# deep-art-project/Music

Hardware: AMD Instinct MI355X
Metric: audio samples/sec trained (whole node), 30-layer WaveNet @16kHz (higher is better)
Workload: dtype f32 (forward + recompute: f16 2-term split operands, 2^-22 per element; backward products: bf16 2-term split, 2^-17 per element, f32 range; 3 MFMA per product, f32 accumulate)

## Files before the change

### include/wavenet_hip.h

```cpp
#ifndef WAVENET_HIP_H
#define WAVENET_HIP_H
#include <stdint.h>
#ifdef __cplusplus
extern "C" {
#endif

typedef void* wn_stream_t;
enum { WN_F16X3 = 0, WN_F16X1 = 1, WN_BF16X3 = 2, WN_BF16X1 = 3 };
#define WN_ABI_VERSION 9
#define WN_CE_NUM_PARTIALS 1024
#define WN_GUARD_NUM_PARTIALS 256
#define WN_GUARD_PARTIALS_BYTES (WN_GUARD_NUM_PARTIALS * 12)
#define WN_GUARD_STATE_BYTES 48

int wn_version(void);
const char* wn_last_error(void);

int wn_pack_weights(const float* flat, const int32_t* idx, uint16_t* out, int n, int mode,
                    wn_stream_t stream);

int wn_chan_gemm(const float* in0, const float* in1, int64_t in_bstride, int in_pitch, int in_lo, int in_hi,
                 int shift0, int shift1, int ks0, int ks1, const uint16_t* wpack, int mt, int m_valid,
                 float* out, int64_t out_bstride, int out_pitch, int out_shift, const float* bias,
                 const float* resid, int64_t resid_bstride, int resid_pitch, int resid_lo,
// ... 27 lines not shown

int wn_enc_resblock_fwd(const float* x_in, float* x_out, float* h_out, int64_t x_bstride, int64_t h_bstride, int pitch,
                        const uint16_t* wdil, const uint16_t* wd, const float* bias_dil, const float* bias_d, int n_h,
                        int n_d, int ch, int d, int t_lo, int t_hi, int batch, int mode, wn_stream_t stream);

int wn_enc_resblock_bwd(const float* x_in, const float* dy, const float* h, float* dh, int64_t x_bstride,
                        int64_t h_bstride, int64_t dh_bstride, int pitch, const uint16_t* wdT, int ch, int d, int t_lo,
                        int t_hi, int y_lo, float* slab_dil, float* slab_d, int batch, int mode_bwd, wn_stream_t stream);
int wn_enc_resblock_bwd_slabs(int t_lo, int t_hi, int batch);
int wn_enc_resblock_bwd_pq(const float* x_in, const float* p_in, const float* q_in, int dn, int p_lo, const float* h,
                           float* p_out, float* q_out, int64_t x_bstride, int64_t h_bstride, int pitch, const uint16_t* wdT,
                           const uint16_t* wpq, int ch, int d, int t_lo, int t_hi, float* slab_dil, float* slab_d, int chain,
                           int batch, int mode_bwd, wn_stream_t stream);

int wn_resblock_bwd_ms(const float* x_in, const float* dy, const float* dz, float* dfg, int64_t x_bstride,
                       int64_t dz_bstride, int64_t dfg_bstride, int pitch, const uint16_t* wfg, const uint16_t* wdT,
                       const float* bias_f, const float* bias_g, int n_f, int ch, int d, int t_lo, int t_hi, int z_lo,
                       float* slab_fg, float* slab_d, const float* cond, int64_t cond_bstride, int cond_pitch,
                       int cond_mode, int cond_le, int cond_q, int batch, int mode_fwd, int mode_bwd,
                       wn_stream_t stream);
int wn_resblock_bwd_ms_slabs(int t_lo, int t_hi, int batch);

#define WN_COND_IDX_PAD 64
int wn_resblock_bwd_pq(const float* x_in, const float* p_in, const float* q_in, int dn, int p_lo, const float* dz,
                       float* p_out, float* q_out, int64_t x_bstride, int64_t dz_bstride, int pitch, const uint16_t* wfg,
                       const uint16_t* wdT, const uint16_t* wpq, int ch, int d, int t_lo, int t_hi, int z_lo,
                       float* slab_fg, float* slab_d, const float* cond, int64_t cond_bstride, int cond_pitch, int cond_le,
                       const uint8_t* cond_idx, float* cslab, int64_t dz_half_stride, int chain, int batch, int mode_fwd,
                       int mode_bwd, wn_stream_t stream);
int wn_resblock_bwd_pq_chain_ok(int t_lo, int t_hi, int batch, int d);
int wn_resblock_bwd_pq_slabs(int t_lo, int t_hi, int batch, int d, int chain);
int wn_resblock_bwd_pq_chain_items(int t_lo, int t_hi, int batch, int d, int wg, int* out, int cap);
int wn_resblock_bwd_pq_cond_floats(int t_lo, int t_hi, int batch);
int wn_resblock_bwd_pq_cond_reduce(const float* cslab, const int64_t* slab_off, const int* t_lo, int n_launches, int t_hi, int batch,
                                   int cond_le, float* out, int64_t out_lstride, int64_t out_bstride, int out_pitch,
                                   wn_stream_t stream);
int wn_gate_fwd(const float* fg, int64_t fg_bstride, int dp, int rows, float* z, int64_t z_bstride, int pitch, int t_lo, int t_hi,
                int batch, wn_stream_t stream);
int wn_gate_bwd(const float* fg, int64_t fg_bstride, int dp, int rows, const float* dz, int64_t dz_bstride, float* dfg,
                int64_t dfg_bstride, int pitch, int t_lo, int t_hi, int batch, wn_stream_t stream);
int wn_chunk_softmax_fwd(const float* x, float* y, int64_t nrows, int q, wn_stream_t stream);
int wn_chunk_softmax_bwd(const float* y, const float* dy, float* dx, int64_t nrows, int q, wn_stream_t stream);
int wn_chunk_softmax_ce(const float* x, const int64_t* target, float* probs, float* dx, float* loss_part, int64_t nrows, int q,
                        float inv_n, wn_stream_t stream);
int wn_split16(const float* x, uint16_t* hi, uint16_t* lo, int64_t n, int is_bf16, wn_stream_t stream);
int wn_shift_add(const float* p, const float* q, float* out, int64_t bstride, int pitch, int rows, int dn, int p_lo,
                 int t_lo, int t_hi, int batch, wn_stream_t stream);

int wn_wgrad(const float* a, int64_t a_bstride, int a_pitch, int a_shift, int a_cols,
             const float* b0, const float* b1, int64_t b_bstride, int b_pitch, int b_shift0,
             int b_shift1, int b_cols, int nt_per_tap, int mt, int relu_b, float* c, int ldc,
             int64_t c_slab_stride, int t_lo, int t_hi, int chunk, int batch, int mode, wn_stream_t stream);
int wn_wgrad_slabs(int t_lo, int t_hi, int chunk, int batch);
int wn_causal_wgrad_codes(const int32_t* codes, int scrambled, const float* dx, const float* dx_q, int dn, int p_lo,
                          int64_t dx_bstride, int pitch, int ch, int q, int t, int batch, float* slab, wn_stream_t stream);
int wn_causal_wgrad_codes_slabs(int t, int batch);
int wn_causal_fwd_codes(const int32_t* codes, int scrambled, const float* wt, const float* bias, int n_rows, float* x0,
                        int64_t x_bstride, int pitch, int ch, int q, int t, int batch, wn_stream_t stream);
int wn_reduce_slabs(const int64_t* desc, int n_ops, int64_t total_vec, const float* slab, float* out,
                    wn_stream_t stream);

int wn_bias_grad(const float* a, int64_t a_bstride, int a_pitch, int a_shift, int rows, int t_lo,
                 int t_hi, int batch, float* out, wn_stream_t stream);

int wn_chunk_softmax256_fwd(const float* x, float* y, int64_t nrows, wn_stream_t stream);
int wn_chunk_softmax256_bwd(const float* y, const float* dy, float* dx, int64_t nrows, wn_stream_t stream);
int wn_chunk_softmax256_ce(const float* x, const int64_t* target, float* probs, float* dx,
                           float* loss_part, int64_t nrows, float inv_n, wn_stream_t stream);

int wn_adam_flat(float* p, const float* g, float* m, float* v, int64_t n, float lr, float beta1,
                 float beta2, float eps, float bias_corr1, float bias_corr2, float gscale,
                 wn_stream_t stream);
int wn_sgd_flat(float* p, const float* g, float* momentum_buf, int64_t n, float lr, float momentum, float gscale,
                int first_step, wn_stream_t stream);
int wn_rmsprop_flat(float* p, const float* g, float* square_avg, float* momentum_buf, int64_t n, float lr, float alpha,
                    float eps, float momentum, float gscale, wn_stream_t stream);
typedef struct wn_guard_state {
    float norm;
    float coef;
    uint32_t nonfinite;
    uint32_t skip;
    uint64_t n_taken;
    uint64_t n_clipped;
    uint64_t n_skipped;
    float bc1;
    float bc2;
} wn_guard_state;
int wn_grad_guard(const float* g, int64_t n, float gscale, float max_norm, int skip_nonfinite, float beta1, float beta2,
                  void* partials, wn_guard_state* state, wn_stream_t stream);
int wn_adam_flat_guarded(float* p, const float* g, float* m, float* v, int64_t n, float lr, float beta1, float beta2, float eps,
                         float gscale, const wn_guard_state* state, wn_stream_t stream);
int wn_sgd_flat_guarded(float* p, const float* g, float* momentum_buf, int64_t n, float lr, float momentum, float gscale,
                        const wn_guard_state* state, wn_stream_t stream);
int wn_rmsprop_flat_guarded(float* p, const float* g, float* square_avg, float* momentum_buf, int64_t n, float lr, float alpha,
                            float eps, float momentum, float gscale, const wn_guard_state* state, wn_stream_t stream);
int wn_ema_flat(float* ema, const float* p, int64_t n, float decay, int warmup, int64_t t, const wn_guard_state* state,
                wn_stream_t stream);
int wn_step_softmax(const float* x, int64_t x_bstride, int x_pitch, float* probs, int w, int q, int batch, wn_stream_t stream);
int wn_step_nll(const float* x, int64_t x_bstride, int x_pitch, const int64_t* target, float* dx, int64_t dx_bstride, int dx_pitch,
                float* probs, float* row_nll, int32_t* row_hit, float* loss_part, int w, int q, int batch, float inv_n,
                wn_stream_t stream);
int wn_win_step_softmax(const float* x, int64_t x_bstride, int x_pitch, float* probs, int w, int q, int batch, const int32_t* win_host,
                        int win_period, const int64_t* win_pos, int64_t win_pos0, wn_stream_t stream);
int wn_win_step_nll(const float* x, int64_t x_bstride, int x_pitch, const int64_t* target, float* dx, int64_t dx_bstride, int dx_pitch,
                    float* probs, float* row_nll, int32_t* row_hit, float* loss_part, int w, int q, int batch, float inv_n,
                    const int32_t* win_host, int win_period, const int64_t* win_pos, int64_t win_pos0, wn_stream_t stream);
// ... 155 lines not shown
```

### music_amd/_lib.py

```python
import ctypes
import os

_HERE = os.path.dirname(os.path.abspath(__file__))
LIB_PATH = os.environ.get("WAVENET_HIP_LIB") or os.path.join(_HERE, "libwavenet_hip.so")

F16X3, F16X1, BF16X3, BF16X1 = 0, 1, 2, 3
MODE_NAMES = {"f16x3": F16X3, "f16x1": F16X1, "bf16x3": BF16X3, "bf16x1": BF16X1}
CE_NUM_PARTIALS = 1024
ABI_VERSION = 9
GUARD_NUM_PARTIALS = 256
GUARD_PARTIALS_BYTES = GUARD_NUM_PARTIALS * 12
VQ_NUM_PARTIALS = 256
VQ_MAX_CODES, VQ_MAX_WIDTH = 1024, 512
VQ_EMA_WORK_BYTES = 16 + 4 * VQ_MAX_CODES
RVQ_MAX_STAGES = 8
GCOND_MAX_CHANNELS = 512

_p = ctypes.c_void_p
_i = ctypes.c_int
_l = ctypes.c_int64
_f = ctypes.c_float
_DEC_HEAD = [_i] * 5 + [_p] * 6 + [_l] + [_p] * 12 + [_l, _i, _i, _p]
_DEC_BATCH = [_i, _l, _f, _l]
_DEC_PK = [_p] + [_l] * 6
_DEC_COND = [_p, _l, _p, _l, _p, _p, _i, _l]
_DEC_SAMP = [_p, _i, _f]
_DEC_WIN = [_p, _i, _l]
_SAMPLE_LOGITS = [_p, _l, _i, _l, _p, _f, _l, _i, _f, _l, _p, _p, _p]

SIGNATURES = {
    "wn_version": [],
    "wn_pack_weights": [_p, _p, _p, _i, _i, _p],
    "wn_chan_gemm": [_p, _p, _l, _i, _i, _i, _i, _i, _i, _i, _p, _i, _i,
                     _p, _l, _i, _i, _p,
                     _p, _l, _i, _i,
                     _p, _l, _i,
                     _i, _i, _i, _i, _i, _p],
    "wn_skip_epilogue_fwd": [_p, _l, _i, _i, _p, _p, _p, _p, _l, _p, _p, _p, _p, _p, _l, _i, _i, _i, _i, _i, _i, _i, _p],
    "wn_skip_epilogue_bwd": [_p, _l, _i, _p, _p, _l, _i, _p, _p, _p, _l, _p, _p, _p, _i, _i, _i, _i, _i, _i, _i, _p],
    "wn_resblock_fwd": [_p, _p, _p, _l, _l, _i, _p, _p, _p, _p, _p, _i, _i, _i, _i,
                        _i, _i, _i, _i, _p, _l, _i, _i, _i, _i, _p, _l, _p, _l, _i, _i, _p],
    "wn_enc_resblock_fwd": [_p, _p, _p, _l, _l, _i, _p, _p, _p, _p, _i, _i, _i, _i, _i, _i, _i, _i, _p],
    "wn_enc_resblock_bwd": [_p, _p, _p, _p, _l, _l, _l, _i, _p, _i, _i, _i, _i, _i, _p, _p, _i, _i, _p],
    "wn_enc_resblock_bwd_slabs": [_i, _i, _i],
    "wn_enc_resblock_bwd_pq": [_p, _p, _p, _i, _i, _p, _p, _p, _l, _l, _i, _p, _p, _i, _i, _i, _i, _p, _p, _i, _i, _i, _p],
    "wn_avgpool": [_p, _l, _i, _i, _i, _i, _i, _p, _l, _i, _i, _p],
    "wn_resblock_bwd": [_p, _p, _p, _p, _p, _l, _l, _l, _l, _i, _p, _p, _p, _p, _i, _i, _i, _i, _i, _i,
                        _p, _l, _i, _i, _i, _i, _i, _i, _i, _p],
    "wn_cond_expand": [_p, _l, _i, _i, _i, _i, _i, _i, _i, _p, _l, _i, _i, _p],
    "wn_cond_grad": [_p, _l, _i, _i, _i, _i, _i, _i, _i, _p, _l, _i, _i, _p],
    "wn_avgpool_bwd": [_p, _l, _i, _i, _i, _i, _i, _p, _l, _i, _i, _i, _p],
    "wn_wgrad": [_p, _l, _i, _i, _i, _p, _p, _l, _i, _i, _i, _i, _i, _i, _i, _p, _i,
                 _l, _i, _i, _i, _i, _i, _p],
    "wn_wgrad_slabs": [_i, _i, _i, _i],
    "wn_resblock_bwd_ms": [_p, _p, _p, _p, _l, _l, _l, _i, _p, _p, _p, _p, _i, _i, _i, _i, _i, _i, _p, _p,
                           _p, _l, _i, _i, _i, _i, _i, _i, _i, _p],
    "wn_resblock_bwd_ms_slabs": [_i, _i, _i],
    "wn_resblock_bwd_pq": [_p, _p, _p, _i, _i, _p, _p, _p, _l, _l, _i, _p, _p, _p, _i, _i, _i, _i, _i, _p, _p,
                           _p, _l, _i, _i, _p, _p, _l, _i, _i, _i, _i, _p],
    "wn_resblock_bwd_pq_chain_ok": [_i, _i, _i, _i],
    "wn_resblock_bwd_pq_slabs": [_i, _i, _i, _i, _i],
    "wn_resblock_bwd_pq_chain_items": [_i, _i, _i, _i, _i, _p, _i],
    "wn_resblock_bwd_pq_cond_floats": [_i, _i, _i],
    "wn_resblock_bwd_pq_cond_reduce": [_p, _p, _p, _i, _i, _i, _i, _p, _l, _l, _i, _p],
    "wn_split16": [_p, _p, _p, _l, _i, _p],
    "wn_shift_add": [_p, _p, _p, _l, _i, _i, _i, _i, _i, _i, _i, _p],
    "wn_causal_wgrad_codes": [_p, _i, _p, _p, _i, _i, _l, _i, _i, _i, _i, _i, _p, _p],
    "wn_causal_wgrad_codes_slabs": [_i, _i],
    "wn_causal_fwd_codes": [_p, _i, _p, _p, _i, _p, _l, _i, _i, _i, _i, _i, _p],
    "wn_reduce_slabs": [_p, _i, _l, _p, _p, _p],
    "wn_bias_grad": [_p, _l, _i, _i, _i, _i, _i, _i, _p, _p],
    "wn_chunk_softmax256_fwd": [_p, _p, _l, _p],
    "wn_chunk_softmax256_bwd": [_p, _p, _p, _l, _p],
    "wn_chunk_softmax256_ce": [_p, _p, _p, _p, _p, _l, _f, _p],
    "wn_gate_fwd": [_p, _l, _i, _i, _p, _l, _i, _i, _i, _i, _p],
    "wn_gate_bwd": [_p, _l, _i, _i, _p, _l, _p, _l, _i, _i, _i, _i, _p],
    "wn_chunk_softmax_fwd": [_p, _p, _l, _i, _p],
    "wn_chunk_softmax_bwd": [_p, _p, _p, _l, _i, _p],
    "wn_chunk_softmax_ce": [_p, _p, _p, _p, _p, _l, _i, _f, _p],
    "wn_adam_flat": [_p, _p, _p, _p, _l, _f, _f, _f, _f, _f, _f, _f, _p],
    "wn_sgd_flat": [_p, _p, _p, _l, _f, _f, _f, _i, _p],
    "wn_rmsprop_flat": [_p, _p, _p, _p, _l, _f, _f, _f, _f, _f, _p],
    "wn_grad_guard": [_p, _l, _f, _f, _i, _f, _f, _p, _p, _p],
    "wn_adam_flat_guarded": [_p, _p, _p, _p, _l, _f, _f, _f, _f, _f, _p, _p],
    "wn_sgd_flat_guarded": [_p, _p, _p, _l, _f, _f, _f, _p, _p],
    "wn_rmsprop_flat_guarded": [_p, _p, _p, _p, _l, _f, _f, _f, _f, _f, _p, _p],
    "wn_ema_flat": [_p, _p, _l, _f, _i, _l, _p, _p],
    "wn_step_softmax": [_p, _l, _i, _p, _i, _i, _i, _p],
    "wn_step_nll": [_p, _l, _i, _p, _p, _l, _i, _p, _p, _p, _p, _i, _i, _i, _f, _p],
    "wn_win_step_softmax": [_p, _l, _i, _p, _i, _i, _i, _p, _i, _p, _l, _p],
    "wn_win_step_nll": [_p, _l, _i, _p, _p, _l, _i, _p, _p, _p, _p, _i, _i, _i, _f, _p, _i, _p, _l, _p],
    "wn_cond_proj_fwd": [_p, _p, _l, _l, _l, _l, _l, _p, _p, _p, _i, _i, _i, _i, _i, _i, _i, _p],
    "wn_cond_proj_bwd": [_p, _i, _p, _p, _p, _l, _l, _l, _l, _l, _p, _p, _i, _i, _i, _i, _i, _i, _i, _p],
    "wn_gcond_proj_fwd": [_p, _p, _l, _l, _l, _l, _l, _p, _p, _p, _i, _i, _i, _i, _i, _i, _i, _p, _l, _l, _l, _l, _i, _i, _p],
    "wn_gcond_proj_bwd": [_p, _i, _p, _p, _p, _l, _l, _l, _l, _l, _p, _p, _i, _i, _i, _i, _i, _i, _i, _p, _l, _l, _l, _l, _i, _i, _p],
    "wn_vq_fwd": [_p, _p, _l, _p, _p, _p, _p, _i, _i, _i, _i, _p],
    "wn_vq_bwd": [_p, _p, _p, _p, _l, _f, _f, _p, _p, _i, _i, _i, _i, _p],
    "wn_vq_lookup": [_p, _p, _l, _p, _p, _i, _i, _i, _i, _p],
    "wn_vq_bwd_stats": [_p, _p, _p, _p, _l, _f, _f, _p, _p, _p, _i, _i, _i, _i, _p],
    "wn_vq_ema_update": [_p, _l, _p, _p, _p, _p, _i, _i, _f, _f, _f, _p, _p],
    "wn_rvq_fwd": [_p, _p, _l, _p, _p, _p, _p, _p, _i, _i, _i, _i, _i, _p],
    "wn_rvq_bwd": [_p, _p, _p, _p, _p, _l, _f, _f, _p, _p, _i, _i, _i, _i, _i, _p],
    "wn_rvq_bwd_stats": [_p, _p, _p, _p, _p, _l, _f, _f, _p, _p, _p, _i, _i, _i, _i, _i, _p],
    "wn_rvq_ema_update": [_p, _l, _p, _p, _p, _p, _i, _i, _i, _f, _f, _f, _p, _p],
    "wn_rvq_lookup": [_p, _p, _l, _p, _p, _i, _i, _i, _i, _i, _i, _p],
    "wn_rvq_fwd_n": [_p, _p, _l, _p, _p, _p, _p, _p, _p, _i, _i, _i, _i, _i, _p],
    "wn_rvq_bwd_n": [_p, _p, _p, _p, _p, _p, _l, _f, _f, _p, _p, _i, _i, _i, _i, _i, _p],
# ... 85 lines not shown
def thread_budget(quota, local_world, cpus=None):
    total = quota if quota is not None else (cpus if cpus is not None else (os.cpu_count() or 1))
    return max(1, -(-int(total) // max(1, int(local_world))))


def respect_cpu_quota():
    import sys
    import torch
    if os.environ.get("WN_KEEP_TORCH_THREADS", "0") == "1":
        return
    q, lw = cpu_quota(), local_world_size()
    if q is None and lw == 1:
        return
    n = thread_budget(q, lw)
    if torch.get_num_threads() > n:
        print("music_amd: torch intra-op threads %d -> %d (%s shared by %d rank(s) of this host; WN_KEEP_TORCH_THREADS=1 keeps torch's "
              "own setting)" % (torch.get_num_threads(), n, "the container's CPU quota of %d" % q if q is not None else
                                "%d CPUs" % (os.cpu_count() or 1), lw), file=sys.stderr)
        torch.set_num_threads(n)


def load():
    global _lib
    if _lib is not None:
        return _lib
    if not os.path.exists(LIB_PATH):
        raise WavenetHipError(
            "libwavenet_hip.so not found at %s - build it with `python -c 'import __graft_entry__ as g; "
            "g.build()'` or `make -C music_amd/csrc`; there is no CPU fallback" % LIB_PATH)
    import torch
    lib = ctypes.CDLL(LIB_PATH)
    for name, args in SIGNATURES.items():
        try:
            fn = getattr(lib, name)
        except AttributeError:
            raise WavenetHipError("%s does not export %s: it was built from older sources - rebuild it (`make -C music_amd/csrc`)"
                                  % (LIB_PATH, name)) from None
        fn.argtypes = args
        fn.restype = ctypes.c_int
    lib.wn_decode_sync_granules.restype = ctypes.c_int64
    lib.wn_last_error.argtypes = []
    lib.wn_last_error.restype = ctypes.c_char_p
    if lib.wn_version() != ABI_VERSION:
        raise WavenetHipError("libwavenet_hip.so ABI version %d != expected %d" % (lib.wn_version(), ABI_VERSION))
    _lib = lib
    respect_cpu_quota()
    return lib


def wgrad_slabs(t_lo, t_hi, chunk, batch):
    return load().wn_wgrad_slabs(t_lo, t_hi, chunk, batch)


def causal_codes_slabs(t, batch):
    return load().wn_causal_wgrad_codes_slabs(t, batch)


COND_IDX_PAD = 64


def ms_slabs(t_lo, t_hi, batch):
    return load().wn_resblock_bwd_ms_slabs(t_lo, t_hi, batch)


def pq_chain_ok(t_lo, t_hi, batch, d):
    return bool(load().wn_resblock_bwd_pq_chain_ok(t_lo, t_hi, batch, d))


def pq_slabs(t_lo, t_hi, batch, d, chain):
    return load().wn_resblock_bwd_pq_slabs(t_lo, t_hi, batch, d, 1 if chain else 0)


def enc_slabs(t_lo, t_hi, batch):
    return load().wn_enc_resblock_bwd_slabs(t_lo, t_hi, batch)


def decode_sync_granules(n_layers, D, S):
    return int(load().wn_decode_sync_granules(n_layers, D, S))


def call(name, *args):
    lib = load()
    rc = getattr(lib, name)(*args)
    if rc != 0:
        raise WavenetHipError("%s failed (%d): %s" % (name, rc, lib.wn_last_error().decode()))


def ptr(t, offset=0):
    if t is None:
        return None
    return t.data_ptr() + offset * t.element_size()


def stream():
    import torch
    return torch.cuda.current_stream().cuda_stream


_side_streams = {}


def side_stream(device):
    import os
    import torch
    dev = torch.device(device)
    key = dev.index if dev.index is not None else torch.cuda.current_device()
# ... 5 lines not shown
```

### music_amd/csrc/wn_api.hip

```cpp
#include <stdio.h>
#include <stdlib.h>
#include <string.h>
#include "../../include/wavenet_hip.h"
#include "wn_common.h"
#include "wn_kernels.h"

static_assert(WN_COND_IDX_PAD == WN_PQ_IDX_PAD, "public and kernel-side pad of the bucket bytes differ");
static thread_local char g_err[512] = "";

int wn_set_error(hipError_t e, const char* file, int line) {
    snprintf(g_err, sizeof(g_err), "HIP error %d (%s) at %s:%d", (int)e, hipGetErrorString(e), file, line);
    return -1;
}
int wn_tile_origin(int t_lo) { return t_lo & ~63; }

int wn_num_cus() {
    static std::atomic<int> cus{0};
    int v = cus.load(std::memory_order_relaxed);
    if (v > 0) return v;
    int dev = 0;
    hipDeviceProp_t pr;
    if (hipGetDevice(&dev) != hipSuccess || hipGetDeviceProperties(&pr, dev) != hipSuccess || pr.multiProcessorCount <= 0) return 256;
    cus.store(pr.multiProcessorCount, std::memory_order_relaxed);
    return pr.multiProcessorCount;
// ... 247 lines not shown
        if (write_x) WN_REQUIRE("wn_resblock_fwd", x_out);
    }
    WnResArgs a;
    memset(&a, 0, sizeof(a));
    a.x_in = x_in; a.x_out = x_out; a.z_out = z_out; a.x_bstride = x_bstride; a.z_bstride = z_bstride; a.pitch = pitch;
    a.wfg = wfg; a.wd = wd; a.bias_f = bias_f; a.bias_g = bias_g; a.bias_d = bias_d; a.n_f = n_f; a.n_d = n_d;
    a.d = d; a.t_lo = t_lo; a.t_hi = t_hi; a.z_lo = z_lo; a.write_x = write_x;
    a.cond = cond; a.cond_bstride = cond_bstride; a.cond_pitch = cond_pitch; a.cond_mode = cond_mode;
    a.cond_le = cond_le; a.cond_q = cond_q;
    if (cond && cond_pack && cond_idx) { a.cond_pack = cond_pack; a.cond_pack_bstride = cond_pack_bstride; a.cond_idx = cond_idx; }
    if (z_half_stride && ch != 64) return wn_set_error_msg(-4, "wn_resblock_fwd: z_half_stride is for two 32-channel clips on the 64-channel block");
    a.z_half = z_half_stride;
    return wn_launch_resblock_fwd(a, ch, batch, mode, (hipStream_t)stream);
}

int wn_resblock_bwd(const float* x_in, const float* dy, const float* dz, float* dfg, float* z,
                    int64_t x_bstride, int64_t dz_bstride, int64_t dfg_bstride, int64_t z_bstride,
                    int pitch, const uint16_t* wfg, const uint16_t* wdT, const float* bias_f,
                    const float* bias_g, int n_f, int ch, int d, int t_lo, int t_hi, int z_lo,
                    const float* cond, int64_t cond_bstride, int cond_pitch, int cond_mode, int cond_le, int cond_q,
                    int batch, int mode_fwd, int mode_bwd, wn_stream_t stream) {
    if (pitch % 4 != 0) return wn_set_error_msg(-4, "wn_resblock_bwd: pitch must be a multiple of 4");
    if (batch > 0 && t_hi > t_lo) {
        WN_REQUIRE("wn_resblock_bwd", x_in, dz, dfg, wfg);
        if (dy) WN_REQUIRE("wn_resblock_bwd", wdT);
    }
    WnResBwdArgs a;
    memset(&a, 0, sizeof(a));
    a.x_in = x_in; a.dy = dy; a.dz = dz; a.dfg = dfg; a.z = z;
    a.x_bstride = x_bstride; a.dz_bstride = dz_bstride; a.dfg_bstride = dfg_bstride; a.z_bstride = z_bstride; a.pitch = pitch;
    a.wfg = wfg; a.wdT = wdT; a.bias_f = bias_f; a.bias_g = bias_g; a.n_f = n_f;
    a.d = d; a.t_lo = t_lo; a.t_hi = t_hi; a.z_lo = z_lo;
    a.cond = cond; a.cond_bstride = cond_bstride; a.cond_pitch = cond_pitch; a.cond_mode = cond_mode;
    a.cond_le = cond_le; a.cond_q = cond_q;
    return wn_launch_resblock_bwd(a, ch, batch, mode_fwd, mode_bwd, (hipStream_t)stream);
}

int wn_wgrad(const float* a_, int64_t a_bstride, int a_pitch, int a_shift, int a_cols,
             const float* b0, const float* b1, int64_t b_bstride, int b_pitch, int b_shift0,
             int b_shift1, int b_cols, int nt_per_tap, int mt, int relu_b, float* c, int ldc,
             int64_t c_slab_stride, int t_lo, int t_hi, int chunk, int batch, int mode, wn_stream_t stream) {
    if (c_slab_stride < (int64_t)mt * 16 * ldc) return wn_set_error_msg(-4, "wn_wgrad: slab stride smaller than C");
    if (batch > 0 && t_hi > t_lo) WN_REQUIRE("wn_wgrad", a_, b0, c);
    WnWgradArgs a;
    memset(&a, 0, sizeof(a));
    a.a = a_; a.a_bstride = a_bstride; a.a_pitch = a_pitch; a.a_shift = a_shift; a.a_cols = a_cols;
    a.b0 = b0; a.b1 = b1; a.b_bstride = b_bstride; a.b_pitch = b_pitch; a.b_shift0 = b_shift0; a.b_shift1 = b_shift1; a.b_cols = b_cols;
    a.nt_per_tap = nt_per_tap; a.mt = mt; a.relu_b = relu_b; a.c = c; a.ldc = ldc; a.c_slab_stride = c_slab_stride;
    a.t_lo = t_lo; a.t_hi = t_hi; a.chunk = chunk;
    return wn_launch_wgrad(a, batch, mode, (hipStream_t)stream);
}

int wn_wgrad_slabs(int t_lo, int t_hi, int chunk, int batch) { return wn_wgrad_num_slabs(t_lo, t_hi, chunk, batch); }

int wn_reduce_slabs(const int64_t* desc, int n_ops, int64_t total_vec, const float* slab, float* out, wn_stream_t stream) {
    if (n_ops > 0 && total_vec > 0) WN_REQUIRE("wn_reduce_slabs", desc, slab, out);
    return wn_launch_reduce_slabs(reinterpret_cast<const long*>(desc), n_ops, total_vec, slab, out, (hipStream_t)stream);
}

int wn_bias_grad(const float* a, int64_t a_bstride, int a_pitch, int a_shift, int rows, int t_lo,
                 int t_hi, int batch, float* out, wn_stream_t stream) {
    if (batch > 0 && t_hi > t_lo && rows > 0) WN_REQUIRE("wn_bias_grad", a, out);
    return wn_launch_bias_grad(a, a_bstride, a_pitch, a_shift, rows, t_lo, t_hi, batch, out, (hipStream_t)stream);
}

int wn_chunk_softmax256_fwd(const float* x, float* y, int64_t nrows, wn_stream_t stream) {
    if (nrows > 0) WN_REQUIRE("wn_chunk_softmax256_fwd", x, y);
    return wn_launch_softmax_fwd(x, y, nrows, (hipStream_t)stream);
}
int wn_chunk_softmax256_bwd(const float* y, const float* dy, float* dx, int64_t nrows, wn_stream_t stream) {
    if (nrows > 0) WN_REQUIRE("wn_chunk_softmax256_bwd", y, dy, dx);
    return wn_launch_softmax_bwd(y, dy, dx, nrows, (hipStream_t)stream);
}
int wn_chunk_softmax256_ce(const float* x, const int64_t* target, float* probs, float* dx,
                           float* loss_part, int64_t nrows, float inv_n, wn_stream_t stream) {
    if (nrows > 0) WN_REQUIRE("wn_chunk_softmax256_ce", x, target);
    return wn_launch_softmax_ce(x, target, probs, dx, loss_part, nrows, inv_n, (hipStream_t)stream);
}
int wn_adam_flat(float* p, const float* g, float* m, float* v, int64_t n, float lr, float beta1,
                 float beta2, float eps, float bias_corr1, float bias_corr2, float gscale, wn_stream_t stream) {
    if (n > 0) WN_REQUIRE("wn_adam_flat", p, g, m, v);
    return wn_launch_adam(p, g, m, v, n, lr, beta1, beta2, eps, bias_corr1, bias_corr2, gscale, (hipStream_t)stream);
}
int wn_sgd_flat(float* p, const float* g, float* momentum_buf, int64_t n, float lr, float momentum, float gscale, int first_step,
                wn_stream_t stream) {
    if (momentum != 0.f && !momentum_buf) return wn_set_error_msg(-4, "wn_sgd_flat: momentum needs its buffer");
    if (n > 0) WN_REQUIRE("wn_sgd_flat", p, g);
    return wn_launch_sgd(p, g, momentum_buf, n, lr, momentum, gscale, first_step, (hipStream_t)stream);
}
int wn_rmsprop_flat(float* p, const float* g, float* square_avg, float* momentum_buf, int64_t n, float lr, float alpha, float eps,
                    float momentum, float gscale, wn_stream_t stream) {
    if (!square_avg || (momentum > 0.f && !momentum_buf)) return wn_set_error_msg(-4, "wn_rmsprop_flat: missing state buffer");
    if (n > 0) WN_REQUIRE("wn_rmsprop_flat", p, g);
    return wn_launch_rmsprop(p, g, square_avg, momentum_buf, n, lr, alpha, eps, momentum, gscale, (hipStream_t)stream);
}

int wn_grad_guard(const float* g, int64_t n, float gscale, float max_norm, int skip_nonfinite, float beta1, float beta2, void* partials,
                  wn_guard_state* state, wn_stream_t stream) {
    WN_REQUIRE("wn_grad_guard", partials, state);
    if (n > 0) WN_REQUIRE("wn_grad_guard", g);
    if (n < 0) return wn_set_error_msg(-4, "wn_grad_guard: n is negative");
    if (((uintptr_t)g & 3) || ((uintptr_t)partials & 7) || ((uintptr_t)state & 7))
        return wn_set_error_msg(-4, "wn_grad_guard: g needs 4-byte, partials and state 8-byte alignment");
    return wn_launch_grad_guard(g, n, gscale, max_norm, skip_nonfinite, beta1, beta2, partials, state, (hipStream_t)stream);
}
int wn_adam_flat_guarded(float* p, const float* g, float* m, float* v, int64_t n, float lr, float beta1, float beta2, float eps,
// ... 695 lines not shown
```

### music_amd/csrc/wn_kernels.h

```cpp
#pragma once
#include <hip/hip_runtime.h>
#include <stdint.h>

enum { WN_MODE_F16X3 = 0, WN_MODE_F16X1 = 1, WN_MODE_BF16X3 = 2, WN_MODE_BF16X1 = 3 };
static inline int wn_mode_is_bf16(int m) { return m >= 2; }
static inline int wn_mode_ns(int m) { return (m & 1) ? 1 : 3; }
static inline size_t wn_frag_halfs(int mode) { return wn_mode_ns(mode) == 3 ? 1024 : 512; }

struct WnGemmArgs {
    const float* in0; const float* in1;
    long in_bstride; int in_pitch; int in_lo, in_hi;
    int shift0, shift1;
    int ks0, ks1;
    const uint16_t* wpack;
    int mt, m_valid;
    float* out; long out_bstride; int out_pitch; int out_shift;
    const float* bias;
    const float* resid; long resid_bstride; int resid_pitch; int resid_lo;
    const float* mask; long mask_bstride; int mask_pitch;
    int t_lo, t_hi, t_base;
    int relu_in;
    int swz;
};
int wn_launch_gemm(const WnGemmArgs& a, int batch, int mode, hipStream_t st);
// ... 90 lines not shown
    const uint16_t* wfg; const uint16_t* wdT; const uint16_t* wpq;
    float* slab_fg; float* slab_d;
    int d, t_lo, t_hi, z_lo, t_base;
    int steps_per_clip, items_per_wg, batch;
    int swz;
    const float* cond; long cond_bstride; int cond_pitch; int cond_le;
    const uint8_t* cond_idx; float* cslab; int cslab_slots;
    long dz_half;
    int chain, ch_s, ch_qn, ch_rm, ch_g, ch_nchain;
};
#define WN_PQ_IDX_PAD 64
int wn_launch_resblock_bwd_pq(const WnResPqArgs& a, int batch, hipStream_t st);
int wn_pq_chain_ok(int t_lo, int t_hi, int batch, int d);
void wn_pq_chain_plan(int t_lo, int t_hi, int batch, int d, int& t_base, int& steps, int& s, int& qn, int& rm, int& g, int& nchain, int& nwg);
int wn_pq_slabs(int t_lo, int t_hi, int batch, int d, int chain);
int wn_pq_chain_items(int t_lo, int t_hi, int batch, int d, int wg, int* out, int cap);
int wn_pq_cond_slots(int t_lo, int t_hi, int batch);
int wn_pq_cond_slab_floats(int t_lo, int t_hi, int batch);
int wn_launch_pq_cond_reduce(const float* cslab, const long* off, const int* t_lo, int n, int t_hi, int batch, int le, float* out,
                             long out_lstride, long out_bstride, int out_pitch, hipStream_t st);
int wn_launch_split16(const float* x, uint16_t* hi, uint16_t* lo, long n, int is_bf16, hipStream_t st);
int wn_launch_shift_add(const float* p, const float* q, float* out, long bstride, int pitch, int rows, int dn,
                        int p_lo, int t_lo, int t_hi, int batch, hipStream_t st);
int wn_launch_enc_bwd_rw(const WnResMsArgs& a, int ch, int batch, int mode_bwd, hipStream_t st);
int wn_enc_bwd_slabs(int t_lo, int t_hi, int batch);
struct WnEncPqArgs {
    const float* x_in;
    const float* p_in; const float* q_in; int dn, p_lo;
    const float* h; long h_bstride;
    float* p_out; float* q_out;
    long x_bstride; int pitch;
    const uint16_t* wdT; const uint16_t* wpq;
    float* slab_dil; float* slab_d;
    int d, t_lo, t_hi, t_base;
    int steps_per_clip, items_per_wg, batch, swz;
    int chain, ch_s, ch_qn, ch_rm, ch_g, ch_nchain;
};
int wn_launch_enc_bwd_pq(const WnEncPqArgs& a, int ch, int batch, int mode_bwd, hipStream_t st);

struct WnWgradArgs {
    const float* a; long a_bstride; int a_pitch; int a_shift; int a_cols;
    const float* b0; const float* b1; long b_bstride; int b_pitch; int b_shift0, b_shift1; int b_cols;
    int nt_per_tap;
    int mt;
    int relu_b;
    float* c; int ldc;
    long c_slab_stride;
    int t_lo, t_hi, t_base; int chunk;
    int swz;
};
int wn_launch_wgrad(const WnWgradArgs& a, int batch, int mode, hipStream_t st);
int wn_launch_wgrad2(const WnWgradArgs* a1, const WnWgradArgs* a2, int batch, int mode, hipStream_t st);
int wn_wgrad_num_slabs(int t_lo, int t_hi, int chunk, int batch);
int wn_launch_reduce_slabs(const long* desc, int n_ops, long total_vec, const float* slab, float* out, hipStream_t st);

int wn_launch_causal_wgrad_codes(const int32_t* codes, int scrambled, const float* dx, const float* dxq, int dn, int p_lo,
                                 long dx_bstride, int pitch, int ch, int T, int batch, float* slab, hipStream_t st);
int wn_causal_codes_slabs(int T, int batch);
int wn_launch_causal_fwd_codes(const int32_t* codes, int scrambled, const float* wt, const float* bias, int n_rows, float* x0,
                               long x_bstride, int pitch, int ch, int T, int batch, hipStream_t st);

int wn_launch_softmax_fwd(const float* x, float* y, long nrows, hipStream_t st);
int wn_launch_softmax_bwd(const float* y, const float* dy, float* dx, long nrows, hipStream_t st);
#define WN_CE_PARTIALS 1024
int wn_launch_softmax_ce(const float* x, const int64_t* target, float* probs, float* dx,
                         float* loss_part, long nrows, float inv_n, hipStream_t st);
int wn_launch_adam(float* p, const float* g, float* m, float* v, long n, float lr, float b1, float b2,
                   float eps, float bc1, float bc2, float gscale, hipStream_t st);
int wn_launch_sgd(float* p, const float* g, float* buf, long n, float lr, float momentum, float gscale, int first, hipStream_t st);
int wn_launch_rmsprop(float* p, const float* g, float* sq, float* buf, long n, float lr, float alpha, float eps, float momentum,
                      float gscale, hipStream_t st);
struct wn_guard_state;
int wn_launch_grad_guard(const float* g, long n, float gscale, float max_norm, int skip_nonfinite, float beta1, float beta2,
                         void* partials, wn_guard_state* state, hipStream_t st);
int wn_launch_adam_guarded(float* p, const float* g, float* m, float* v, long n, float lr, float b1, float b2, float eps, float gscale,
                           const wn_guard_state* state, hipStream_t st);
int wn_launch_sgd_guarded(float* p, const float* g, float* buf, long n, float lr, float momentum, float gscale,
                          const wn_guard_state* state, hipStream_t st);
int wn_launch_rmsprop_guarded(float* p, const float* g, float* sq, float* buf, long n, float lr, float alpha, float eps, float momentum,
                              float gscale, const wn_guard_state* state, hipStream_t st);
int wn_launch_ema(float* ema, const float* p, long n, float decay, int warmup, long t, const wn_guard_state* state, hipStream_t st);
int wn_launch_gather_grads(const float* packed, const int32_t* idx, float* flat_grad, int n, hipStream_t st);
int wn_launch_gather_grads2(const float* packed, const int32_t* idx, const int32_t* idx2, float* flat_grad, int n, hipStream_t st);
int wn_launch_onehot(const int32_t* idx, float* out, int batch, int q, int t, int scrambled, hipStream_t st);
int wn_launch_mulaw_encode(const float* audio, const float* thr, uint8_t* codes, long n, hipStream_t st);
int wn_launch_mulaw_decode(const uint8_t* codes, const float* table, float* audio, long n, hipStream_t st);
int wn_launch_mulaw_encode_q(const float* audio, const float* thr, int n_thr, int32_t* codes, long n, hipStream_t st);
int wn_launch_mulaw_decode_q(const int32_t* codes, const float* table, int q, float* audio, long n, hipStream_t st);
int wn_launch_bias_grad(const float* a, long a_bstride, int a_pitch, int a_shift, int rows, int t_lo,
                        int t_hi, int batch, float* out, hipStream_t st);

int wn_launch_cond_expand(const float* tab, long tab_bstride, int tab_pitch, int rows, int t_lo, int t_hi, int mode, int le, int q,
                          float* out, long out_bstride, int out_pitch, int batch, hipStream_t st);
int wn_launch_cond_grad(const float* in, long in_bstride, int in_pitch, int rows, int t_lo, int t_hi, int mode, int le,
                        int q, float* out, long out_bstride, int out_pitch, int batch, hipStream_t st);
int wn_launch_avgpool_bwd(const float* denc, long denc_bstride, int denc_pitch, int t0, int pool, int n_out, int rows,
                          float* out, long out_bstride, int out_pitch, int t_hi, int batch, hipStream_t st);
int wn_launch_avgpool(const float* in, long in_bstride, int in_pitch, int t0, int pool, int n_out, int rows,
                      float* out, long out_bstride, int out_pitch, int batch, hipStream_t st);

struct WnCondProj {
    const float* enc; const float* flat;
    long w_off, b_off, stage_stride, wf_off, bf_off;
    float* tab; float* tab_pair; float* enf;
    const float* d_tab; int d_pair; const float* d_enf; float* d_enc; float* flat_grad;
    int n_stages, dd, ch, sd, bw, le, batch;
// ... 99 lines not shown
```

### music_amd/csrc/wn_wgrad.hip

```cpp
#include <type_traits>
#include "wn_common.h"
#include "wn_kernels.h"

struct WgRaw { f32x4 u0, u1; };

__device__ __forceinline__ WgRaw wg_load(const float* row, int col, int ncols) {
    WgRaw r;
    r.u0 = ld4g(row + col, col, 0, ncols);
    r.u1 = ld4g(row + col + 4, col + 4, 0, ncols);
    return r;
}

template <class T, int NS>
__device__ __forceinline__ void wg_frag(Frag<T>& f, const WgRaw& r, int t, int t_lo, int t_hi, bool masked, bool relu) {
    float v[8] = {r.u0[0], r.u0[1], r.u0[2], r.u0[3], r.u1[0], r.u1[1], r.u1[2], r.u1[3]};
    if (masked) {
#pragma unroll
        for (int j = 0; j < 8; ++j)
            if (t + j < t_lo || t + j >= t_hi) v[j] = 0.f;
    }
    if (relu) {
#pragma unroll
        for (int j = 0; j < 8; ++j) v[j] = fmaxf(v[j], 0.f);
    }
    split8<T, NS>(f, v);
}

struct WnWgradPair { WnWgradArgs p[2]; int y_split; };

template <class T, int NS>
__global__ __launch_bounds__(512) void wgrad_k(WnWgradPair pr) {
    __shared__ float red[4][64 * 64];
    const WnBlock wb = wn_block(pr.p[0].swz);
    const bool second = wb.y >= pr.y_split;
    const WnWgradArgs& a = pr.p[second ? 1 : 0];
    const int by = second ? wb.y - pr.y_split : wb.y;
    const int lane = threadIdx.x & 63, wave = __builtin_amdgcn_readfirstlane(threadIdx.x >> 6);
    const int c = lane & 15, q = lane >> 4;
    const int b = wb.z;
    const int nt_total = a.nt_per_tap * (a.b1 ? 2 : 1);
    const int nblk_n = (nt_total + 3) / 4, nblk_m = (a.mt + 3) / 4;
    const int nblk = nblk_n * nblk_m;
    const bool split_time = nblk == 1;
    const int blk = split_time ? 0 : by * 4 + (wave & 3);
    const bool active = blk < nblk;
    const int mb = active ? blk / nblk_n : 0, nb = active ? blk % nblk_n : 0;
    int tc0 = a.t_base + wb.x * a.chunk;
    int tc1 = tc0 + a.chunk;
    if (tc1 > a.t_hi) tc1 = a.t_hi;
    const int n_chunks = (a.t_hi - a.t_base + a.chunk - 1) / a.chunk;
    {
        const int ts = split_time ? 8 : 2, part = split_time ? wave : (wave >> 2);
// ... 220 lines not shown
            park(0, tc0);
            issue(tc0 + 32 < tc1 ? tc0 + 32 : tb_last);
        }
        __syncthreads();
        int it = 0;
        for (int tb = tc0; tb < tc1; tb += 32, ++it) {
            const int tb1 = tb + 32 < tc1 ? tb + 32 : tb_last, tb2 = tb + 64 < tc1 ? tb + 64 : tb_last;
            const uint16_t* base = l_f + (size_t)(it & 1) * 32 * FR;
            Frag<T> bf[4], af[2];
#pragma unroll
            for (int n = 0; n < 4; ++n) load_a<T, NS>(bf[n], base, 16 + wn * 4 + n, lane);
            load_a<T, NS>(af[0], base, wm * 8, lane);
#pragma unroll
            for (int m = 0; m < 8; ++m) {
                if (m + 1 < 8) load_a<T, NS>(af[(m + 1) & 1], base, wm * 8 + m + 1, lane);
                if (m == 4) {
                    __builtin_amdgcn_sched_barrier(0);
                    park((it + 1) & 1, tb1);
                    __builtin_amdgcn_sched_barrier(0);
                }
                if (m >= 4) {
                    issue_piece(tb2, m - 4, 0);
                    issue_piece(tb2, m - 4, 1);
                }
#pragma unroll
                for (int n = 0; n < 4; ++n) mma<T, NS>(acc[m][n], af[m & 1], bf[n]);
                __builtin_amdgcn_sched_barrier(0);
            }
            __syncthreads();
        }
    };
    {
        const int last_tb = tc0 + ((tc1 - 1 - tc0) & ~31);
        if (tc0 >= tb_lo && last_tb <= tb_hi) run(std::false_type{});
        else run(std::true_type{});
    }
    const int n_chunks = (a.t_hi - a.t_base + a.chunk - 1) / a.chunk;
    float* cs = a.c + ((size_t)b * n_chunks + wb.x) * a.c_slab_stride;
#pragma unroll
    for (int m = 0; m < 8; ++m) {
        const int mt = mg * 16 + wm * 8 + m;
        if (mt >= a.mt) continue;
#pragma unroll
        for (int n = 0; n < 4; ++n) {
            const int nt = ng * 16 + wn * 4 + n;
            if (nt >= nt_total) continue;
#pragma unroll
            for (int i = 0; i < 4; ++i)
                cs[(size_t)(mt * 16 + 4 * q + i) * a.ldc + nt * 16 + c] = acc[m][n][i];
        }
    }
}

static void wg_prepare(WnWgradArgs& k, int& nchunks, int& ygroups) {
    k.t_base = k.t_lo & ~31;
    k.swz = wn_xcd_swizzle_enabled();
    if (k.chunk < 128) k.chunk = 128;
    k.chunk = (k.chunk + 127) & ~127;
    const int nt_total = k.nt_per_tap * (k.b1 ? 2 : 1);
    const int nblk = ((nt_total + 3) / 4) * ((k.mt + 3) / 4);
    nchunks = (k.t_hi - k.t_base + k.chunk - 1) / k.chunk;
    ygroups = (nblk + 3) / 4;
}

int wn_launch_wgrad2(const WnWgradArgs* a1, const WnWgradArgs* a2, int batch, int mode, hipStream_t st) {
    if (batch <= 0) return 0;
    WnWgradPair pr;
    int n = 0, nch[2] = {0, 0}, yg[2] = {0, 0};
    const WnWgradArgs* src[2] = {a1, a2};
    for (int i = 0; i < 2; ++i) {
        if (!src[i] || src[i]->t_hi <= src[i]->t_lo) continue;
        pr.p[n] = *src[i];
        wg_prepare(pr.p[n], nch[n], yg[n]);
        ++n;
    }
    if (n == 0) return 0;
    if (n == 1) {
        const WnWgradArgs& k = pr.p[0];
        const int nt_total = k.nt_per_tap * (k.b1 ? 2 : 1);
        if (k.mt >= 16 && nt_total >= 16) {
            const int ns = wn_mode_ns(mode);
            const size_t sh = (size_t)2 * 32 * (ns == 3 ? 1024 : 512) * sizeof(uint16_t);
            dim3 g(nch[0], ((k.mt + 15) / 16) * ((nt_total + 15) / 16), batch), b(512);
            int dev = 0;
            (void)hipGetDevice(&dev);
            static WnDevOnce done[4];
#define WN_BIG(TT, NN, slot) do { \
                if (done[slot].need(dev)) { \
                    (void)hipFuncSetAttribute(reinterpret_cast<const void*>(&wgrad_big_k<TT, NN>), \
                                              hipFuncAttributeMaxDynamicSharedMemorySize, (int)sh); \
                    done[slot].done(dev); } \
                hipLaunchKernelGGL((wgrad_big_k<TT, NN>), g, b, sh, st, k); } while (0)
            switch (mode) {
                case WN_MODE_BF16X3: WN_BIG(BF16, 3, 0); break;
                case WN_MODE_BF16X1: WN_BIG(BF16, 1, 1); break;
                case WN_MODE_F16X3: WN_BIG(F16, 3, 2); break;
                case WN_MODE_F16X1: WN_BIG(F16, 1, 3); break;
                default: return wn_set_error_msg(-2, "wgrad: bad mode");
            }
#undef WN_BIG
            WN_CHECK_LAUNCH();
            return 0;
        }
        pr.p[1] = pr.p[0]; yg[1] = 0; nch[1] = 0;
    }
    pr.y_split = yg[0];
    dim3 g(nch[0] > nch[1] ? nch[0] : nch[1], yg[0] + yg[1], batch), b(512);
    switch (mode) {
        case WN_MODE_BF16X3: hipLaunchKernelGGL((wgrad_k<BF16, 3>), g, b, 0, st, pr); break;
        case WN_MODE_BF16X1: hipLaunchKernelGGL((wgrad_k<BF16, 1>), g, b, 0, st, pr); break;
        case WN_MODE_F16X3: hipLaunchKernelGGL((wgrad_k<F16, 3>), g, b, 0, st, pr); break;
        case WN_MODE_F16X1: hipLaunchKernelGGL((wgrad_k<F16, 1>), g, b, 0, st, pr); break;
        default: return wn_set_error_msg(-2, "wgrad: bad mode");
    }
    WN_CHECK_LAUNCH();
    return 0;
}

int wn_launch_wgrad(const WnWgradArgs& a, int batch, int mode, hipStream_t st) {
    return wn_launch_wgrad2(&a, nullptr, batch, mode, st);
}

__global__ __launch_bounds__(256) void reduce_slabs_k(const long* __restrict__ desc, int n_ops, long total_vec,
                                                      const float* __restrict__ slab, float* __restrict__ out) {
    long v = (long)blockIdx.x * blockDim.x + threadIdx.x;
    if (v >= total_vec) return;
    int lo = 0, hi = n_ops - 1;
    while (lo < hi) {
        int mid = (lo + hi + 1) >> 1;
        if (desc[mid * 6] <= v) lo = mid; else hi = mid - 1;
    }
    const long* d = desc + lo * 6;
    const long e = (v - d[0]) * 4, n = d[5], stride = d[3];
    const int ns = (int)d[2];
    const float* sp = slab + d[1] + e;
    float* op = out + d[4] + e;
    if (e + 3 < n) {
        f32x4 s8[8];
// ... 30 lines not shown
```

Measured before the change: 31.27 million.

## Add specialized row-tiled wgrad kernel for 256-row single-tap weight gradients

Adds a dedicated weight-gradient kernel for the case mt==16, single B operand, and 3-term split modes. Each of the 8 waves owns two N tiles and all 16 M tiles, so the A operand is split and staged in a 4-stage LDS ring shared across waves. B fragments stay in registers, and global loads are software-pipelined with the MFMA loop. The aim is to cut redundant A splitting and global traffic and to improve latency hiding versus the generic big kernel. In exchange it uses 128 KB of LDS and a large accumulator array (32 f32x4), which may limit occupancy or spill registers. It is enabled by default and can be switched off with an environment variable or an API toggle.

```diff
diff --git a/include/wavenet_hip.h b/include/wavenet_hip.h
--- a/include/wavenet_hip.h
+++ b/include/wavenet_hip.h
@@ -103,6 +103,7 @@
              int b_shift1, int b_cols, int nt_per_tap, int mt, int relu_b, float* c, int ldc,
              int64_t c_slab_stride, int t_lo, int t_hi, int chunk, int batch, int mode, wn_stream_t stream);
 int wn_wgrad_slabs(int t_lo, int t_hi, int chunk, int batch);
+int wn_wgrad_select(int form);
 int wn_causal_wgrad_codes(const int32_t* codes, int scrambled, const float* dx, const float* dx_q, int dn, int p_lo,
                           int64_t dx_bstride, int pitch, int ch, int q, int t, int batch, float* slab, wn_stream_t stream);
 int wn_causal_wgrad_codes_slabs(int t, int batch);
diff --git a/music_amd/_lib.py b/music_amd/_lib.py
--- a/music_amd/_lib.py
+++ b/music_amd/_lib.py
@@ -53,6 +53,7 @@
     "wn_wgrad": [_p, _l, _i, _i, _i, _p, _p, _l, _i, _i, _i, _i, _i, _i, _i, _p, _i,
                  _l, _i, _i, _i, _i, _i, _p],
     "wn_wgrad_slabs": [_i, _i, _i, _i],
+    "wn_wgrad_select": [_i],
     "wn_resblock_bwd_ms": [_p, _p, _p, _p, _l, _l, _l, _i, _p, _p, _p, _p, _i, _i, _i, _i, _i, _i, _p, _p,
                            _p, _l, _i, _i, _i, _i, _i, _i, _i, _p],
     "wn_resblock_bwd_ms_slabs": [_i, _i, _i],
@@ -244,6 +245,10 @@
     return load().wn_wgrad_slabs(t_lo, t_hi, chunk, batch)
 
 
+def wgrad_select(form):
+    return load().wn_wgrad_select(form)
+
+
 def causal_codes_slabs(t, batch):
     return load().wn_causal_wgrad_codes_slabs(t, batch)
 
diff --git a/music_amd/csrc/wn_api.hip b/music_amd/csrc/wn_api.hip
--- a/music_amd/csrc/wn_api.hip
+++ b/music_amd/csrc/wn_api.hip
@@ -323,6 +323,7 @@
 }
 
 int wn_wgrad_slabs(int t_lo, int t_hi, int chunk, int batch) { return wn_wgrad_num_slabs(t_lo, t_hi, chunk, batch); }
+int wn_wgrad_select(int form) { return wn_wgrad_rows_select(form); }
 
 int wn_reduce_slabs(const int64_t* desc, int n_ops, int64_t total_vec, const float* slab, float* out, wn_stream_t stream) {
     if (n_ops > 0 && total_vec > 0) WN_REQUIRE("wn_reduce_slabs", desc, slab, out);
diff --git a/music_amd/csrc/wn_kernels.h b/music_amd/csrc/wn_kernels.h
--- a/music_amd/csrc/wn_kernels.h
+++ b/music_amd/csrc/wn_kernels.h
@@ -166,6 +166,7 @@
 int wn_launch_wgrad(const WnWgradArgs& a, int batch, int mode, hipStream_t st);
 int wn_launch_wgrad2(const WnWgradArgs* a1, const WnWgradArgs* a2, int batch, int mode, hipStream_t st);
 int wn_wgrad_num_slabs(int t_lo, int t_hi, int chunk, int batch);
+int wn_wgrad_rows_select(int form);
 int wn_launch_reduce_slabs(const long* desc, int n_ops, long total_vec, const float* slab, float* out, hipStream_t st);
 
 int wn_launch_causal_wgrad_codes(const int32_t* codes, int scrambled, const float* dx, const float* dxq, int dn, int p_lo,
diff --git a/music_amd/csrc/wn_wgrad.hip b/music_amd/csrc/wn_wgrad.hip
--- a/music_amd/csrc/wn_wgrad.hip
+++ b/music_amd/csrc/wn_wgrad.hip
@@ -1,3 +1,4 @@
+#include <stdlib.h>
 #include <type_traits>
 #include "wn_common.h"
 #include "wn_kernels.h"
@@ -324,6 +325,140 @@
     }
 }
 
+template <class T>
+__global__ __launch_bounds__(512) void wgrad_rows_k(WnWgradArgs a) {
+    constexpr int NS = 3, FR = 1024, ST = 16 * FR;
+    extern __shared__ __attribute__((aligned(16))) uint16_t l_a[];
+    const int lane = threadIdx.x & 63, wave = __builtin_amdgcn_readfirstlane(threadIdx.x >> 6);
+    const int c = lane & 15, q = lane >> 4;
+    const WnBlock wb = wn_block<true>(a.swz);
+    const int b = wb.z;
+    const int nt_total = a.nt_per_tap;
+    const int ng = wb.y;
+    const int tc0 = a.t_base + wb.x * a.chunk;
+    int tc1 = tc0 + a.chunk;
+    if (tc1 > a.t_hi) tc1 = a.t_hi;
+
+    const float* arow[2];
+    const float* brow[2];
+    bool bval[2];
+#pragma unroll
+    for (int k = 0; k < 2; ++k) {
+        arow[k] = a.a + (size_t)b * a.a_bstride + (size_t)((2 * wave + k) * 16) * a.a_pitch;
+        const int nt = ng * 16 + 2 * wave + k;
+        bval[k] = nt < nt_total;
+        brow[k] = a.b0 + (size_t)b * a.b_bstride + (size_t)((bval[k] ? nt : 0) * 16) * a.b_pitch;
+    }
+    const bool work = bval[0];
+    const int aoff = c * a.a_pitch + 8 * q, boff = c * a.b_pitch + 8 * q;
+    f32x4 acc[16][2];
+#pragma unroll
+    for (int m = 0; m < 16; ++m)
+#pragma unroll
+        for (int n = 0; n < 2; ++n) acc[m][n] = f32x4{0.f, 0.f, 0.f, 0.f};
+
+    WgRaw ra[2], rb[2];
+    Frag<T> bf0[2], bf1[2];
+    const bool relu = a.relu_b != 0;
+    const int tb_lo = -min(a.a_shift, a.b_shift0);
+    const int tb_hi = min(a.a_cols - a.a_shift, a.b_cols - a.b_shift0) - 32;
+    const int tb_last = tc0 + ((tc1 - 1 - tc0) & ~31);
+    auto clampt = [&](int tb) { return tb < tc1 ? tb : tb_last; };
+    auto park_a = [&](int k, int s, int tb) {
+        const bool masked = (tb < a.t_lo) || (tb + 32 > tc1);
+        Frag<T> f;
+        wg_frag<T, NS>(f, ra[k], tb + 8 * q, a.t_lo, tc1, masked, false);
+        u32x4* dst = reinterpret_cast<u32x4*>(l_a + (size_t)(s & 3) * ST + (size_t)(2 * wave + k) * FR);
+        dst[lane] = __builtin_bit_cast(u32x4, f.hi);
+        dst[64 + lane] = __builtin_bit_cast(u32x4, f.lo);
+    };
+    auto split_b = [&](Frag<T>& f, int n, int tb) {
+        const bool masked = (tb < a.t_lo) || (tb + 32 > tc1) || !bval[n];
+        wg_frag<T, NS>(f, rb[n], tb + 8 * q, a.t_lo, tc1, masked, relu);
+    };
+    auto run = [&](auto guarded) {
+        auto load = [&](WgRaw& r, const float* tile, int off, int pitch, int shift, int cols, int tb) {
+            if (decltype(guarded)::value) {
+                r = wg_load(tile + c * pitch, tb + 8 * q + shift, cols);
+            } else {
+                const float* p = tile + (tb + shift) + off;
+                r.u0 = ld4u(p);
+                r.u1 = ld4u(p + 4);
+            }
+        };
+        auto load_a2 = [&](int k, int tb) { load(ra[k], arow[k], aoff, a.a_pitch, a.a_shift, a.a_cols, tb); };
+        auto load_b = [&](int n, int tb) { load(rb[n], brow[n], boff, a.b_pitch, a.b_shift0, a.b_cols, tb); };
+        if (tc0 >= tc1) return;
+        {
+            const int t1 = clampt(tc0 + 32), t2 = clampt(tc0 + 64);
+            load_a2(0, tc0); load_a2(1, tc0); load_b(0, tc0); load_b(1, tc0);
+            park_a(0, 0, tc0); park_a(1, 0, tc0);
+            load_a2(0, t1); load_a2(1, t1);
+            split_b(bf0[0], 0, tc0); split_b(bf0[1], 1, tc0);
+            load_b(0, t1); load_b(1, t1);
+            park_a(0, 1, t1); park_a(1, 1, t1);
+            load_a2(0, t2); load_a2(1, t2);
+        }
+        __syncthreads();
+        auto step = [&](int s, int tb, Frag<T> (&cur)[2], Frag<T> (&nxt)[2]) {
+            const int tb1 = clampt(tb + 32), tb2 = clampt(tb + 64), tb3 = clampt(tb + 96);
+            const uint16_t* base = l_a + (size_t)(s & 3) * ST;
+            Frag<T> af[2];
+            if (work) load_a<T, NS>(af[0], base, 0, lane);
+#pragma unroll
+            for (int m = 0; m < 16; ++m) {
+                if (work && m + 1 < 16) load_a<T, NS>(af[(m + 1) & 1], base, m + 1, lane);
+                if (m == 2) split_b(nxt[0], 0, tb1);
+                if (m == 3) load_b(0, tb2);
+                if (m == 4) split_b(nxt[1], 1, tb1);
+                if (m == 5) load_b(1, tb2);
+                if (m == 8) park_a(0, s + 2, tb2);
+                if (m == 9) load_a2(0, tb3);
+                if (m == 10) park_a(1, s + 2, tb2);
+                if (m == 11) load_a2(1, tb3);
+                if (work) {
+#pragma unroll
+                    for (int n = 0; n < 2; ++n) mma<T, NS>(acc[m][n], af[m & 1], cur[n]);
+                }
+            }
+        };
+        for (int s = 0, tb = tc0;;) {
+            step(s, tb, bf0, bf1);
+            ++s; tb += 32;
+            if (tb >= tc1) break;
+            step(s, tb, bf1, bf0);
+            ++s; tb += 32;
+            __syncthreads();
+            if (tb >= tc1) break;
+        }
+    };
+    if (tc0 >= tb_lo && tb_last <= tb_hi) run(std::false_type{});
+    else run(std::true_type{});
+
+    const int n_chunks = (a.t_hi - a.t_base + a.chunk - 1) / a.chunk;
+    float* cs = a.c + ((size_t)b * n_chunks + wb.x) * a.c_slab_stride;
+#pragma unroll
+    for (int m = 0; m < 16; ++m) {
+#pragma unroll
+        for (int n = 0; n < 2; ++n) {
+            const int nt = ng * 16 + 2 * wave + n;
+            if (nt >= nt_total) continue;
+#pragma unroll
+            for (int i = 0; i < 4; ++i)
+                cs[(size_t)(m * 16 + 4 * q + i) * a.ldc + nt * 16 + c] = acc[m][n][i];
+        }
+    }
+}
+
+static std::atomic<int> g_wg_rows{-1};
+int wn_wgrad_rows_select(int form) { return g_wg_rows.exchange(form < 0 ? -1 : (form != 0 ? 1 : 0)); }
+static bool wg_rows_on() {
+    const int f = g_wg_rows.load(std::memory_order_relaxed);
+    if (f >= 0) return f != 0;
+    static const bool env = [] { const char* e = getenv("WN_WGRAD_ROWS"); return e ? atoi(e) != 0 : true; }();
+    return env;
+}
+
 static void wg_prepare(WnWgradArgs& k, int& nchunks, int& ygroups) {
     k.t_base = k.t_lo & ~31;
     k.swz = wn_xcd_swizzle_enabled();
@@ -356,6 +491,20 @@
             dim3 g(nch[0], ((k.mt + 15) / 16) * ((nt_total + 15) / 16), batch), b(512);
             int dev = 0;
             (void)hipGetDevice(&dev);
+            if (k.mt == 16 && !k.b1 && ns == 3 && (mode == WN_MODE_BF16X3 || mode == WN_MODE_F16X3) && wg_rows_on()) {
+                static WnDevOnce rdone[2];
+                const size_t rsh = (size_t)4 * 16 * 1024 * sizeof(uint16_t);
+#define WN_ROWS(TT, slot) do { \
+                if (rdone[slot].need(dev)) { \
+                    (void)hipFuncSetAttribute(reinterpret_cast<const void*>(&wgrad_rows_k<TT>), \
+                                              hipFuncAttributeMaxDynamicSharedMemorySize, (int)rsh); \
+                    rdone[slot].done(dev); } \
+                hipLaunchKernelGGL((wgrad_rows_k<TT>), g, b, rsh, st, k); } while (0)
+                if (mode == WN_MODE_BF16X3) WN_ROWS(BF16, 0); else WN_ROWS(F16, 1);
+#undef WN_ROWS
+                WN_CHECK_LAUNCH();
+                return 0;
+            }
             static WnDevOnce done[4];
 #define WN_BIG(TT, NN, slot) do { \
                 if (done[slot].need(dev)) { \
```

New measurement: 31.44 million (median of 6 runs). No clear change (+0.5%).
